# deflect-ca/banjax

Measured on AMD Instinct MI355X. Metric: log lines/sec matched+rate-limited (node) at 1k rules; HBM GB/s vs peak, higher is better.
Workload: dtype u8

## Files before the change

banjax_amd/csrc/engine.hip:

```cpp
#include <hip/hip_runtime.h>
#include <hipcub/hipcub.hpp>

#include <algorithm>
#include <array>
#include <atomic>
#include <cstdio>
#include <cstdlib>
#include <cstring>
#include <map>
#include <tuple>
#include <memory>
#include <mutex>
#include <stdexcept>
#include <string>
#include <unordered_map>
#include <thread>
#include <vector>

#include "../../include/banjax_gpu.h"
#include "bjx_common.h"
#include "engine_types.h"
#include "regex_compiler.h"
#include "bans.h"
#include "snapshot.h"
// ... 2545 lines not shown
      for (uint32_t w = w0; w < w1; ++w) {
        const uint64_t y = A[w] & cm[w];
        Yb[w] = y;
        for (uint64_t g = y & gall[w]; g; g &= g - 1) {
          const uint32_t gid = aux[w * 64u + (uint32_t)__builtin_ctzll(g)];
          atomicOr(&gmark[gid >> 5], 1u << (gid & 31));
        }
      }
      wide_sync<GLB>();
      if (s_flag) { m = true; break; }
      for (uint32_t w = w0; w < w1; ++w)
        A[w] = ((Yb[w] & sh[w]) << 1) | (w ? (Yb[w - 1] & sh[w - 1]) >> 63 : 0ull) | s0[w];
      wide_sync<GLB>();
      for (uint32_t gi = tid; gi < gw; gi += kBlock) {
        uint32_t mm = gmark[gi];
        if (!mm) continue;
        gmark[gi] = 0;
        for (; mm; mm &= mm - 1) {
          const uint32_t g = gi * 32 + (uint32_t)__ffs(mm) - 1;
          for (uint32_t q = goff[g]; q < goff[g + 1]; ++q)
            atomicOr(reinterpret_cast<unsigned long long *>(&A[gtgt[q] >> 6]), 1ull << (gtgt[q] & 63));
        }
      }
      wide_sync<GLB>();
      if (owner && (A[mw] & mbit)) s_flag = 1;
      wide_sync<GLB>();
      if (s_flag) { m = true; break; }
    }
    if (!m) {
      if (Ly.flags & kNfaAsserts) cross(ctx * 4 + 3);
      wide_sync<GLB>();
      if (owner && (A[mw] & mbit)) s_flag = 1;
      wide_sync<GLB>();
      m = s_flag != 0;
    }
    if (m && tid == 0) {
      const int32_t hid = L.host_id[j];
      atomicOr(reinterpret_cast<unsigned long long *>(&L.mword(j, pos >> 6)), 1ull << (pos & 63));
      atomicAdd(reinterpret_cast<unsigned long long *>(L.counts + j), (1ull << 32) | (is_skip(B, r, hid) ? 0ull : 1ull));
    }
    wide_sync<GLB>();
  }
}

__global__ void k_rule_bounds(uint64_t n, const uint32_t *__restrict__ jkey, uint32_t *__restrict__ first,
                              uint32_t *__restrict__ last) {
  const uint64_t i = (uint64_t)blockIdx.x * blockDim.x + threadIdx.x;
  if (i >= n) return;
  const uint32_t r = jkey[i] & 0xFFFFFF;
  if (i == 0 || (jkey[i - 1] & 0xFFFFFF) != r) first[r] = (uint32_t)i;
  if (i + 1 == n || (jkey[i + 1] & 0xFFFFFF) != r) last[r] = (uint32_t)(i + 1);
}

__global__ __launch_bounds__(kBlock) void k_emit(Bind B, uint64_t n_lines, Lines L, const uint64_t *__restrict__ offs,
                                                 uint64_t *__restrict__ res_seq, uint32_t *__restrict__ res_rule,
                                                 uint32_t *__restrict__ ev_el, uint32_t *__restrict__ ev_rule,
                                                 uint32_t *__restrict__ ev_res, unsigned long long *bounds, bool want_res) {
  __shared__ unsigned long long s_acc[2][kBlock / 64];
  unsigned long long has_ev = 0, ipb = 0;
  for (uint64_t j = (uint64_t)blockIdx.x * blockDim.x + threadIdx.x; j < n_lines; j += (uint64_t)gridDim.x * blockDim.x) {
    const uint64_t cnt = L.counts[j];
    if (cnt == 0) continue;
    uint64_t ro = offs[j] >> 32, eo = offs[j] & 0xFFFFFFFFull;
    const int32_t hid = L.host_id[j];
    uint32_t s_begin = 0, s_end = 0;
    if (hid >= 0) { s_begin = B.site_off[hid]; s_end = B.site_off[hid + 1]; }
    const uint32_t nsite = s_end - s_begin;
    const uint32_t napp = nsite + B.n_global;
    const uint32_t sc = hid >= 0 ? (uint32_t)hid : B.n_hosts;
    const uint64_t k0 = B.sc_skip[2 * sc], k1 = B.sc_skip[2 * sc + 1];
    for (uint32_t w = 0; w * 64 < napp; ++w) {
      uint64_t m = L.mword(j, w);
      while (m) {
        const uint32_t b = (uint32_t)__ffsll((unsigned long long)m) - 1;
        m &= m - 1;
        const uint32_t pos = w * 64 + b;
        const uint32_t r = pos < nsite ? B.site_rules[s_begin + pos] : B.global_rules[pos - nsite];
        const bool skip = pos < 128 ? (((pos < 64 ? k0 >> pos : k1 >> (pos - 64)) & 1) != 0) : is_skip(B, r, hid);
        if (want_res) {
          res_seq[ro] = (j << 16) | pos;
          res_rule[ro] = r | (skip ? 0x80000000u : 0u);
        }
        if (!skip) {
          ev_el[eo] = (uint32_t)j;
          ev_rule[eo] = r;
          if (want_res) ev_res[eo] = (uint32_t)ro;
          ++eo;
        }
        ++ro;
      }
    }
    if (cnt & 0xFFFFFFFFull) { ++has_ev; ipb += L.ip_len[j]; }
  }
  for (int o = 32; o > 0; o >>= 1) {
    has_ev += __shfl_xor(has_ev, o);
    ipb += __shfl_xor(ipb, o);
  }
  if ((threadIdx.x & 63) == 0) { s_acc[0][threadIdx.x >> 6] = has_ev; s_acc[1][threadIdx.x >> 6] = ipb; }
  __syncthreads();
  if (threadIdx.x == 0) {
    unsigned long long a0 = 0, a1 = 0;
    for (int w = 0; w < kBlock / 64; ++w) { a0 += s_acc[0][w]; a1 += s_acc[1][w]; }
    if (a0) { atomicAdd(&bounds[0], a0); atomicAdd(&bounds[1], a1); }
  }
}


__device__ __forceinline__ uint64_t line_start(const uint64_t *nl, uint64_t line) { return line ? nl[line - 1] + 1 : 0; }

__device__ __forceinline__ const uint8_t *ev_ip(const EvSrc &E, uint64_t i) {
  return E.bytes + (E.nl ? line_start(E.nl, i) + E.rest_off[i] - E.ip_len[i] - 1 : E.ip_pos[i]);
}
__device__ __forceinline__ uint64_t ev_hash(const EvSrc &E, uint64_t i, const uint4 &k16, uint32_t len) {
  const uint64_t h = E.nl && len <= 15 ? key16_hash(k16, len) : E.ip_hash[i];
  return E.hmask ? (h & E.hmask) | 1ull : h;
}
// ... 2203 lines not shown
  hipStream_t stream = nullptr;
  hipEvent_t ev0 = nullptr, ev1 = nullptr, evm0 = nullptr, evm1 = nullptr;
  hipEvent_t evk[4] = {};
  double kernel_ms[3] = {};
  uint32_t last_line_kernel = 0;
  static constexpr int kPhases = 8;
  hipEvent_t ph[kPhases + 1] = {};
  double phase_ms[kPhases] = {};
  hipEvent_t xev[2] = {};
  hipStream_t bstream = nullptr;
  hipEvent_t bev[kBanChunks + 1] = {};
  bool xev_rec = false;
  double exchange_ms = 0;
  bool phase_rec[kPhases + 1] = {};

  struct Entry { bool global; std::string site; int32_t decision; std::string ip; };
  std::vector<Entry> decisions;
  uint64_t decisions_version = 1;

  std::unordered_map<std::string, uint32_t> name_ids;
  std::vector<std::string> names;

  uint64_t bound_uid = 0, bound_dec_version = 0;
  DevBuf<uint8_t> bind_blob;
  Bind bind{};
  std::vector<uint4> nfa_rules;
  DevBuf<uint32_t> rb_first, rb_last;
  std::vector<uint32_t> h_first, h_last;
  std::vector<DevRule> host_rules;

  State S{};
  uint64_t ip_cap = 0, st_cap = 0;
  uint64_t ip_cap0 = 0, st_cap0 = 0, arena_cap0 = 0;
  uint64_t rehashes = 0;
  uint64_t last_new_ips = 0, last_new_states = 0;
  uint32_t epoch = 0;
  uint64_t dbg_hash_mask = 0;
  uint64_t dbg_budget = 0;
  uint32_t lines2_lds = 0;
  uint32_t lines2_w = 0;
  int dbg_slot_cache = -1;
  uint64_t host_counters[3] = {0, 0, 0};
  bool counters_fresh = false, want_counters = false;
  static constexpr uint32_t kPinBytes = 16384, kPinReads = 32;
  uint8_t *pin = nullptr;
  uint32_t pin_used = 0, pin_n = 0;
  struct PinRead { void *dst; const uint8_t *slot; uint32_t n; } pin_q[kPinReads];

  DevBuf<uint8_t> staging;
  DevBuf<uint32_t> tile_counts;
  DevBuf<uint64_t> tile_base, nl;
  DevBuf<int64_t> l_ts;
  DevBuf<uint64_t> l_iph, l_counts, l_offs, l_masks;
  DevBuf<uint32_t> l_iplen, l_roff, slow_list;
  DevBuf<int32_t> l_hid;
  DevBuf<uint64_t> l_cand;
  DevBuf<uint4> l_ip16;
  DevBuf<uint32_t> jline, jkey, jidx, jidx2, jkey2;
  DevBuf<uint64_t> jrec;
  uint64_t last_jobs = 0, last_long_runs = 0;
  DevBuf<uint64_t> long_heads;
  DevBuf<uint64_t> lr_end, lr_len, lr_off, lr_win;
  DevBuf<unsigned long long> chk;
  DevBuf<uint64_t> wide_scratch;
  DevBuf<uint32_t> wl_line, wl_rule, wl_pos;
  uint32_t wide_max_w = 0, wide_max_g = 0, n_wide = 0;
  DevBuf<uint32_t> chk_w;
  DevBuf<uint32_t> chk_wb;
  DevBuf<int64_t> lr_t0, lr_h0;
  DevBuf<uint32_t> lr_flags, lr_nwin;
  DevBuf<unsigned long long> long_count;
  DevBuf<uint32_t> bk_start, bk_big, bk_key, bk_pos;
  DevBuf<unsigned long long> bk_nbig;
  DevBuf<uint4> bk_seg;
  DevBuf<EvRec> bk_rec;
  DevBuf<uint8_t> bk_out;
  uint64_t last_big_events = 0;
  uint32_t sort2_hold = 0;
  uint64_t last_grouping = 0;
  uint32_t scan_lds[2] = {0, 0};
  bool lines_attr = false;
  DevBuf<CandMeta> l_ccnt;
  DevBuf<uint64_t> l_cfirst;
  unsigned long long scan_stats[6] = {0, 0, 0, 0, 0, 0};
  uint64_t last_slow = 0;
  DevBuf<uint8_t> l_flags;
  DevBuf<unsigned long long> scalars;
  DevBuf<uint64_t> res_seq;
  bool res_written = false;
  DevBuf<uint32_t> res_rule, ev_el, ev_rule, ev_res, ev_st, ev_st2, ev_idx, ev_idx2, el_slot, coll, trip_idx;
  DevBuf<EvRec> ev_rec, ev_rec2;
  bool rec12 = false;
  int64_t rec_base = 0;
  DevBuf<uint32_t> el_id;
  DevBuf<uint32_t> blk_n;
  DevBuf<uint64_t> blk_b;
  DevBuf<uint8_t> rl_out, ev_out, ev_out_s, trip_flag;
  DevBuf<uint32_t> trip_ev, trip_ev2;
  DevBuf<uint64_t> tr_base;
  DevBuf<bjx_trip> d_trips;
  DevBuf<bjx_rule_result> d_results;
  DevBuf<uint8_t> cub_tmp;
  DevBuf<int64_t> q_out;
  DevBuf<uint8_t> q_ip;

  BatchCtx bc;
// ... 1416 lines not shown
  S.ip_mask = cap - 1;
  (void)hipFree(S.ip_st);
  HIP_OK(hipMalloc(&S.ip_st, cap * 4));
  HIP_OK(hipMemsetAsync(S.ip_st, 0xFF, cap * 4, e->stream));
  S.ip_st_cap = cap;
  e->ip_cap = cap;
  ++e->rehashes;
}

void grow_st(bjx_engine *e, uint64_t want) {
  State &S = e->S;
  const uint64_t cap = next_pow2(want * 4 / 3 + 1024);
  if (cap <= e->st_cap) return;
  StSlot *nt;
  HIP_OK(hipMalloc(&nt, cap * sizeof(StSlot)));
  HIP_OK(hipMemsetAsync(nt, 0, cap * sizeof(StSlot), e->stream));
  hipLaunchKernelGGL(k_rehash_st, dim3(grid_for(e->st_cap)), dim3(kBlock), 0, e->stream, e->st_cap, S.st, nt, cap - 1);
  HIP_OK(hipGetLastError());
  HIP_OK(hipStreamSynchronize(e->stream));
  (void)hipFree(S.st);
  S.st = nt;
  S.st_mask = cap - 1;
  HIP_OK(hipMemsetAsync(S.ip_st, 0xFF, S.ip_st_cap * 4, e->stream));
  if (cap > (1ull << 32)) S.hot_name = kNone;
  e->st_cap = cap;
  ++e->rehashes;
}

void ensure_capacity(bjx_engine *e, uint64_t new_ips, uint64_t new_bytes, uint64_t new_states) {
  State &S = e->S;
  const uint64_t n_ips = e->host_counters[0], used = e->host_counters[1], n_st = e->host_counters[2];
  if ((n_ips + new_ips) * 4 > e->ip_cap * 3) grow_ip(e, 2 * (n_ips + new_ips));
  if (used + new_bytes > S.arena_cap) {
    const uint64_t cap = std::max<uint64_t>(S.arena_cap * 2, used + new_bytes + (1 << 20));
    uint8_t *na;
    HIP_OK(hipMalloc(&na, cap));
    HIP_OK(hipMemcpyAsync(na, S.arena, used, hipMemcpyDeviceToDevice, e->stream));
    HIP_OK(hipStreamSynchronize(e->stream));
    (void)hipFree(S.arena);
    S.arena = na;
    S.arena_cap = cap;
  }
  if ((n_st + new_states) * 4 > e->st_cap * 3) grow_st(e, 2 * (n_st + new_states));
}

template <typename F>
void cub_call(bjx_engine *e, F f) {
  size_t bytes = 0;
  HIP_OK(f((void *)nullptr, bytes));
  e->cub_tmp.ensure(bytes + 16);
  HIP_OK(f((void *)e->cub_tmp.p, bytes));
}

int bit_width(uint64_t x) {
  int b = 0;
  while (x) { ++b; x >>= 1; }
  return b;
}

}

extern "C" int bjx_engine_create(int device, const bjx_engine_options *opts, bjx_engine **out, char *err, size_t err_len) {
  if (!out) return BJX_ERR_ARG;
  *out = nullptr;
  auto e = std::make_unique<bjx_engine>();
  try {
    int n = 0;
    HIP_OK(hipGetDeviceCount(&n));
    if (device < 0 || device >= n) throw BjxError(BJX_ERR_DEVICE, "no such HIP device");
    e->device = device;
    HIP_OK(hipSetDevice(device));
    HIP_OK(hipStreamCreateWithFlags(&e->stream, hipStreamNonBlocking));
    HIP_OK(hipHostMalloc(reinterpret_cast<void **>(&e->pin), bjx_engine::kPinBytes, hipHostMallocDefault));
    HIP_OK(hipEventCreate(&e->ev0));
    HIP_OK(hipEventCreate(&e->ev1));
    HIP_OK(hipEventCreate(&e->evm0));
    HIP_OK(hipEventCreate(&e->evm1));
    for (auto &x : e->evk) HIP_OK(hipEventCreate(&x));
    for (auto &x : e->ph) HIP_OK(hipEventCreate(&x));
    for (auto &x : e->xev) HIP_OK(hipEventCreate(&x));
    uint64_t ipc = std::max<uint64_t>(opts && opts->ip_capacity ? next_pow2(opts->ip_capacity) : 0, 1ull << 22);
    uint64_t stc = std::max<uint64_t>(opts && opts->state_capacity ? next_pow2(opts->state_capacity) : 0, 1ull << 22);
    uint64_t ar = opts && opts->ip_arena_bytes ? opts->ip_arena_bytes : (64ull << 20);
    alloc_state(e.get(), ipc, stc, ar);
    e->ip_cap0 = ipc; e->st_cap0 = stc; e->arena_cap0 = ar;
    *out = e.release();
    return BJX_OK;
  } catch (const BjxError &x) {
    set_err(err, err_len, x.what());
    return x.code;
  }
}

extern "C" void bjx_engine_destroy(bjx_engine *e) {
  if (!e) return;
  (void)hipSetDevice(e->device);
  (void)hipStreamSynchronize(e->stream);
  free_state(e);
  e->trips.release(); e->trips_c.release(); e->d_trips_c.release(); e->results.release(); e->line_flags.release();
  e->ev_out_s.release(); e->trip_ev.release(); e->trip_ev2.release();
  for (auto *b : {&e->staging, &e->l_flags, &e->ev_out, &e->rl_out, &e->trip_flag, &e->bind_blob,
                  &e->cub_tmp, &e->q_ip})
    b->release();
  e->tile_counts.release(); e->tile_base.release(); e->nl.release(); e->l_ts.release(); e->l_iph.release();
  e->l_counts.release(); e->l_offs.release(); e->l_masks.release(); e->l_iplen.release();
  e->l_roff.release(); e->slow_list.release(); e->l_hid.release();
  e->scalars.release(); e->res_seq.release(); e->res_rule.release(); e->ev_el.release(); e->ev_rule.release();

  e->ev_res.release(); e->ev_st.release(); e->ev_st2.release(); e->ev_idx.release(); e->ev_idx2.release();
  e->el_slot.release(); e->coll.release(); e->blk_n.release(); e->blk_b.release(); e->ev_rec.release(); e->ev_rec2.release(); e->el_id.release();

  for (auto *b : {&e->pack_src, &e->rx_len, &e->rx_ev_el}) b->release();
  for (auto *b : {&e->pk_hist, &e->pk_off, &e->pk_counts, &e->pk_bbase, &e->rx_hash, &e->rx_pos, &e->rx_nev, &e->rx_evoff})
    b->release();
  e->rx_ts.release(); e->rx_ip16.release(); e->trip_idx.release(); e->d_trips.release(); e->tr_base.release();
  for (auto *b : {&e->bn_key, &e->bn_key2, &e->bn_len, &e->bn_off, &e->dl_hash}) b->release();
  for (auto *b : {&e->bn_val, &e->bn_val2, &e->bn_head, &e->bn_seg, &e->bn_first, &e->bn_cnt, &e->bn_ipt, &e->bn_coll,
                  &e->dl_off, &e->dl_len, &e->nm_off})
    b->release();
  for (auto *b : {&e->bn_kind, &e->bn_flag, &e->bn_log, &e->dl_bytes, &e->nm_json}) b->release();
  e->bn_best.release(); e->bn_rep.release(); e->bn_sel.release(); e->bn_ipb.release(); e->tz_at.release(); e->tz_off.release();
  e->rb_first.release(); e->rb_last.release(); e->long_heads.release(); e->long_count.release();
  e->lr_end.release(); e->lr_len.release(); e->lr_off.release(); e->lr_win.release(); e->lr_t0.release(); e->lr_h0.release();
  e->lr_flags.release(); e->lr_nwin.release(); e->chk.release(); e->chk_w.release(); e->chk_wb.release();
  for (auto *b : {&e->bk_start, &e->bk_big, &e->bk_key, &e->bk_pos}) b->release();
  e->bk_nbig.release(); e->bk_seg.release(); e->bk_rec.release(); e->bk_out.release();
  e->d_results.release(); e->q_out.release();
  e->ban_ips.release(); e->ban_log.release(); e->ban_off.release(); e->ban_kind.release(); e->ban_ipb.release();
  e->ban_ipo.release();
  e->snap_pin.release();
  e->qry_rows.release();
  e->qry_bytes.release();
  e->l_ip16.release(); e->jline.release(); e->jkey.release(); e->jidx.release(); e->jidx2.release(); e->jrec.release(); e->jkey2.release(); e->l_cand.release(); e->l_ccnt.release(); e->l_cfirst.release();
  (void)hipEventDestroy(e->ev0); (void)hipEventDestroy(e->ev1); (void)hipEventDestroy(e->evm0); (void)hipEventDestroy(e->evm1);
  for (auto &x : e->evk) (void)hipEventDestroy(x);
  for (auto &x : e->ph) (void)hipEventDestroy(x);
  for (auto &x : e->xev) (void)hipEventDestroy(x);
  for (auto &x : e->bev) if (x) (void)hipEventDestroy(x);
  if (e->bstream) (void)hipStreamDestroy(e->bstream);
  (void)hipStreamDestroy(e->stream);
  if (e->pin) (void)hipHostFree(e->pin);
  delete e;
}

extern "C" const char *bjx_engine_last_error(bjx_engine *e) { return e ? e->last_error.c_str() : "no engine"; }

extern "C" int bjx_engine_set_decision_lists(bjx_engine *e, const bjx_decision_entry *entries, size_t n) {
  if (!e || (n && !entries)) return BJX_ERR_ARG;
  std::lock_guard<std::mutex> g(e->mu);
  std::vector<bjx_engine::Entry> v;
  for (size_t i = 0; i < n; ++i) {
    if (entries[i].decision < BJX_ALLOW || entries[i].decision > BJX_IPTABLES_BLOCK) return BJX_ERR_DECISION;
    bjx_engine::Entry x;
    x.global = entries[i].site.ptr == nullptr;
    if (!x.global) x.site.assign(entries[i].site.ptr, entries[i].site.len);
    x.decision = entries[i].decision;
    x.ip.assign(entries[i].ip.ptr ? entries[i].ip.ptr : "", entries[i].ip.len);
    v.push_back(std::move(x));
// ... 376 lines not shown
    const uint8_t *sp = bytes;
    if (flags & BJX_INPUT_DEVICE) {
      sample.resize(sn);
      if (sn) HIP_OK(hipMemcpy(sample.data(), bytes, sn, hipMemcpyDeviceToHost));
      sp = sample.data();
    }
    bind_ruleset(e, rs, sp, sn);
  }
  const Bind &B = e->bind;
  hipStream_t st = e->stream;
  memset(out, 0, sizeof *out);
  e->trips.clear();
  e->trips_c.clear();
  e->results.clear();
  e->line_flags.clear();
  if (n == 0) return false;

  const uint8_t *buf = bytes;
  if (!(flags & BJX_INPUT_DEVICE) || (reinterpret_cast<uintptr_t>(bytes) & 15)) {
    e->staging.ensure(n + 16);
    HIP_OK(hipMemcpyAsync(e->staging.p, bytes, n, (flags & BJX_INPUT_DEVICE) ? hipMemcpyDeviceToDevice : hipMemcpyHostToDevice, st));
    buf = e->staging.p;
  }
  HIP_OK(hipEventRecord(e->ev0, st));
  for (auto &r : e->phase_rec) r = false;
  mark(e, 0);

  const uint64_t n_tiles = (n + kWT - 1) / kWT;
  e->tile_counts.ensure(n_tiles);
  e->tile_base.ensure(n_tiles + 1);
  uint64_t n_lines = 0;
  Lines L;
  hipLaunchKernelGGL(k_nl_count_wt, dim3((unsigned)((n_tiles + 3) / 4)), dim3(kBlock), 0, st, buf, (uint64_t)n, n_tiles,
                     e->tile_counts.p);
  HIP_OK(hipGetLastError());
  {
    uint32_t *in = e->tile_counts.p;
    uint64_t *o = e->tile_base.p;
    cub_call(e, [&](void *tmp, size_t &bytes) { return hipcub::DeviceScan::ExclusiveSum(tmp, bytes, in, o, (int)n_tiles, st); });
  }
  {
    uint64_t last_base = 0;
    uint32_t last_cnt = 0;
    pin_get(e, &last_base, e->tile_base.p + (n_tiles - 1), 8);
    pin_get(e, &last_cnt, e->tile_counts.p + (n_tiles - 1), 4);
    pin_sync(e);
    n_lines = last_base + last_cnt;
  }
  out->n_lines = n_lines;
  if (n_lines == 0) return false;
  const uint64_t cap = n_lines;

  e->nl.ensure(cap);
  e->l_ts.ensure(cap); e->l_iph.ensure(cap); e->l_counts.ensure(cap + 1); e->l_offs.ensure(cap + 1);
  e->l_masks.ensure(cap * B.mask_words);
  e->l_iplen.ensure(cap);
  e->l_roff.ensure(cap); e->l_hid.ensure(cap); e->l_flags.ensure(cap); e->slow_list.ensure(cap);
  e->l_ccnt.ensure(cap); e->l_ip16.ensure(cap);
  e->l_cand.ensure(B.any_prefilter ? cap * kCandSlots : 1);
  e->scalars.ensure(16);
  L.ts = e->l_ts.p; L.ip_hash = e->l_iph.p; L.ip_len = e->l_iplen.p;
  L.rest_off = e->l_roff.p; L.host_id = e->l_hid.p; L.flags = e->l_flags.p;
  L.counts = e->l_counts.p; L.masks = e->l_masks.p; L.mstride = cap;
  L.cand_meta = e->l_ccnt.p; L.cand = e->l_cand.p; L.ip16 = e->l_ip16.p;
  L.cand_first = nullptr;
  if (B.cfirst) {
    e->l_cfirst.ensure(cap * kCandFirstLits);
    L.cand_first = e->l_cfirst.p;
    HIP_OK(hipMemsetAsync(e->l_cfirst.p, 0xFF, cap * kCandFirstLits * 8, st));
  }
  e->jline.ensure(std::max<uint64_t>(e->jline.n, cap + (1u << 20)));
  e->jkey.ensure(e->jline.n); e->jidx.ensure(e->jline.n); e->jrec.ensure(e->jline.n);
  HIP_OK(hipMemsetAsync(e->scalars.p, 0, 16 * sizeof(unsigned long long), st));
  if (B.any_prefilter) HIP_OK(hipMemsetAsync(e->l_ccnt.p, 0, cap * sizeof(CandMeta), st));
  mark(e, 1);

  {
    int n_cu_scan = 0;
    HIP_OK(hipDeviceGetAttribute(&n_cu_scan, hipDeviceAttributeMultiprocessorCount, e->device));
    const unsigned scan_grid = (unsigned)std::min<uint64_t>((n_tiles + kScanWaves - 1) / kScanWaves, (uint64_t)std::max(1, n_cu_scan));
    ScanArgs A;
    A.buf = buf; A.n = n; A.n_tiles = n_tiles; A.n_lines = cap; A.tile_base = e->tile_base.p; A.nl = e->nl.p;
    A.L = L; A.stats = e->scalars.p + 8;
    A.debug_skip = getenv("BJX_DEBUG_SKIP") ? (uint32_t)atoi(getenv("BJX_DEBUG_SKIP")) : 0u;
    const uint32_t fixed = kPairBytes + kScanWaves * kWaveLds;
    const bool img_lds = fixed + B.scan_img_bytes <= kScanLdsMax;
    A.shared_bytes = img_lds ? B.scan_img_bytes : 0;
    const uint32_t lds = A.shared_bytes + kScanWaves * kWaveLds;
    using ScanFn = void (*)(Bind, ScanArgs);
    const ScanFn kfn = img_lds ? k_scan<true> : k_scan<false>;
    if (lds != e->scan_lds[img_lds]) {
      HIP_OK(hipFuncSetAttribute(reinterpret_cast<const void *>(kfn), hipFuncAttributeMaxDynamicSharedMemorySize, (int)lds));
      e->scan_lds[img_lds] = lds;
    }
    HIP_OK(hipEventRecord(e->evm0, st));
    hipLaunchKernelGGL(kfn, dim3(scan_grid), dim3(kScanWaves * 64), lds, st, B, A);
    HIP_OK(hipGetLastError());
    HIP_OK(hipEventRecord(e->evm1, st));
  }
  uint64_t last_nl = 0;
  mark(e, 2);

  unsigned long long sc4[5] = {0, 0, 0, 0, 0};
  unsigned long long n_jobs = 0;
  const bool all_wide = B.n_global > 128 && !(getenv("BJX_LINES") && atoi(getenv("BJX_LINES")) == 1);
  int n_cu = 0;
  HIP_OK(hipDeviceGetAttribute(&n_cu, hipDeviceAttributeMultiprocessorCount, e->device));
// ... 172 lines not shown
        const uint32_t r = k % B.n_rules;
        if (l[k] <= f[k]) continue;
        by_rx[r < rs->rules.size() ? rs->rules[r].regex.substr(0, 60) : "?"] += l[k] - f[k];
        if (k >= B.n_rules) n_legacy += l[k] - f[k];
      }
      std::vector<std::pair<uint64_t, std::string>> v;
      for (auto &kv : by_rx) v.push_back({kv.second, kv.first});
      std::sort(v.rbegin(), v.rend());
      fprintf(stderr, "BJX_JOB_STATS jobs=%llu (legacy %llu) lines=%llu\n", n_jobs, (unsigned long long)n_legacy,
              (unsigned long long)e->bc.n_lines);
      for (size_t i = 0; i < v.size() && i < 16; ++i) fprintf(stderr, "  %10llu  %s\n", (unsigned long long)v[i].first, v[i].second.c_str());
    }
  }
  HIP_OK(hipEventRecord(e->evk[3], st));
  if (n_slow) {
    WideList WL{nullptr, nullptr, nullptr, e->scalars.p + 13, 0};
    if (B.any_wide) {
      const uint64_t cap = n_slow * (uint64_t)e->n_wide + 1;
      e->wl_line.ensure(cap); e->wl_rule.ensure(cap); e->wl_pos.ensure(cap);
      WL.line = e->wl_line.p; WL.rule = e->wl_rule.p; WL.pos = e->wl_pos.p; WL.cap = cap;
      HIP_OK(hipMemsetAsync(e->scalars.p + 13, 0, 8, st));
    }
    if (all_wide) HIP_OK(hipEventRecord(e->evk[0], st));
    hipLaunchKernelGGL(k_parse_match<true>, dim3(grid_for(n_slow)), dim3(kBlock), 0, st, B, buf, e->nl.p, (uint64_t)n_slow,
                       all_wide ? nullptr : e->slow_list.p, now_ns, L, e->slow_list.p, e->scalars.p, WL);
    HIP_OK(hipGetLastError());
    if (B.any_wide) {
      unsigned long long n_wl = 0;
      pin_get(e, &n_wl, e->scalars.p + 13, 8);
      pin_sync(e);
      if (n_wl > WL.cap) throw BjxError(BJX_ERR_DEVICE, "internal: wide-NFA job list overflow");
      if (n_wl) launch_wide(e, B, buf, n, e->wl_rule.p, nullptr, e->wl_line.p, e->wl_pos.p, 0, n_wl, L, e->wide_max_w, e->wide_max_g);
    }
    if (all_wide) HIP_OK(hipEventRecord(e->evk[1], st));
  }
  e->last_slow = n_slow;
  if (getenv("BJX_CHECK")) {
    e->chk.ensure(16);
    HIP_OK(hipMemsetAsync(e->chk.p, 0, 16, st));
    hipLaunchKernelGGL(k_check_masks, dim3(grid_for(n_lines)), dim3(kBlock), 0, st, n_lines, L, B.mask_words, e->chk.p);
    HIP_OK(hipGetLastError());
    unsigned long long c[2];
    pin_get(e, c, e->chk.p, 16);
    pin_sync(e);
    if (c[0]) {
      char msg[160];
      snprintf(msg, sizeof msg, "BJX_CHECK: %llu lines whose RuleResult count differs from their match mask (first %llu)", c[0],
               c[1]);
      throw BjxError(BJX_ERR_DEVICE, msg);
    }
  }
  mark(e, 3);

  HIP_OK(hipMemsetAsync(e->l_counts.p + n_lines, 0, 8, st));
  {
    uint64_t *in = e->l_counts.p, *o = e->l_offs.p;
    cub_call(e, [&](void *tmp, size_t &bytes) {
      return hipcub::DeviceScan::ExclusiveSum(tmp, bytes, in, o, (int)(n_lines + 1), st);
    });
  }
  uint64_t tot = 0;
  pin_get(e, &tot, e->l_offs.p + n_lines, 8);
  pin_sync(e);
  const uint64_t n_res = tot >> 32, n_ev = tot & 0xFFFFFFFFull;
  out->n_results = n_res;
  out->n_events = n_ev;
  e->res_seq.ensure(n_res + 1); e->res_rule.ensure(n_res + 1); e->rl_out.ensure(n_res + 1);
  e->ev_el.ensure(n_ev + 1); e->ev_rule.ensure(n_ev + 1); e->ev_res.ensure(n_ev + 1);
  HIP_OK(hipMemsetAsync(e->scalars.p + 1, 0, 2 * 8, st));
  e->res_written = false;
  if (n_res) {
    const bool want_res = (flags & BJX_COPY_RESULTS) != 0;
    e->res_written = want_res;
    hipLaunchKernelGGL(k_emit, dim3((unsigned)std::min<uint64_t>(grid_for(n_lines), 4096)), dim3(kBlock), 0, st, B, n_lines, L,
                       e->l_offs.p, e->res_seq.p, e->res_rule.p, e->ev_el.p, e->ev_rule.p, e->ev_res.p, e->scalars.p + 1,
                       e->res_written);
    HIP_OK(hipGetLastError());
    if (e->res_written) HIP_OK(hipMemsetAsync(e->rl_out.p, 0, n_res, st));
  }
  mark(e, 4);
  unsigned long long bnd[2] = {0, 0};
  if (n_ev) {
    pin_get(e, bnd, e->scalars.p + 1, 16);
    if (e->want_counters) pin_get(e, e->host_counters, e->S.counters, 24);
    pin_sync(e);
    e->counters_fresh = e->want_counters;
  }
  BatchCtx &c = e->bc;
  c.buf = buf; c.n_lines = n_lines; c.n_res = n_res; c.n_ev = n_ev; c.L = L; c.n_el = bnd[0]; c.el_bytes = bnd[1];
  c.consumed = out->consumed_bytes;
  c.now_ns = now_ns;
  c.live = true;
  return true;
}

static EvSrc local_evsrc(bjx_engine *e) {
  const BatchCtx &c = e->bc;
  EvSrc E;
  E.bytes = c.buf; E.nl = e->nl.p; E.rest_off = c.L.rest_off; E.ip_pos = nullptr; E.ip_len = c.L.ip_len;
  E.ip_hash = c.L.ip_hash; E.ts = c.L.ts; E.counts = c.L.counts; E.ip16 = c.L.ip16; E.n = c.n_lines;
  E.hmask = e->dbg_hash_mask;
  return E;
}

static void ensure_name_json(bjx_engine *e) {
  if (e->nm_built == e->names.size() && e->nm_off.p) return;
  std::vector<uint32_t> off;
  std::vector<uint8_t> js;
  for (const auto &nm : e->names) {
    off.push_back((uint32_t)js.size());
    const uint8_t *b = reinterpret_cast<const uint8_t *>(nm.data());
    JOut<false> c{nullptr, 0};
    json_str(c, b, (uint32_t)nm.size());
    const size_t at = js.size();
    js.resize(at + c.n);
    JOut<true> w{js.data() + at, 0};
    json_str(w, b, (uint32_t)nm.size());
  }
  off.push_back((uint32_t)js.size());
  e->nm_off.ensure(off.size());
  e->nm_json.ensure(js.size() + 16);
  HIP_OK(hipMemcpy(e->nm_off.p, off.data(), off.size() * 4, hipMemcpyHostToDevice));
  if (!js.empty()) HIP_OK(hipMemcpy(e->nm_json.p, js.data(), js.size(), hipMemcpyHostToDevice));
  e->nm_built = e->names.size();
}

__global__ void k_ban_iplen(BanDev A, uint64_t n_ips, const bjx_ip_decision *__restrict__ sel, uint64_t *__restrict__ len) {
  const uint64_t i = (uint64_t)blockIdx.x * blockDim.x + threadIdx.x;
// ... 150 lines not shown
  if (from == kFinSorted)
    hipLaunchKernelGGL(k_trip_events, dim3(grid_for(n_trips)), dim3(kBlock), 0, st, n_trips, e->trip_idx.p, ev_words(e),
                       rec_stride(e), e->trip_ev.p);
  uint32_t *ki = from == kFinSorted ? e->trip_ev.p : e->trip_idx.p, *ko = e->trip_ev2.p;
  const int bits = std::max(1, bit_width(n_ev));
  cub_call(e, [&](void *tmp, size_t &bytes) {
    return hipcub::DeviceRadixSort::SortKeys(tmp, bytes, ki, ko, (int)n_trips, 0, bits, st);
  });
  if (from == kFinList && n_trips > 1) {
    HIP_OK(hipMemsetAsync(e->scalars.p + 6, 0, 8, st));
    hipLaunchKernelGGL(k_count_dups, dim3(grid_for(n_trips)), dim3(kBlock), 0, st, n_trips, ko, e->scalars.p + 6);
    HIP_OK(hipGetLastError());
    unsigned long long dups = 0;
    pin_get(e, &dups, e->scalars.p + 6, 8);
    pin_sync(e);
    if (dups) throw BjxError(BJX_ERR_ARG, "bjx_finish_batch_trips: an event index appears more than once");
  }
  return n_trips;
}

static void finish_phase(bjx_engine *e, uint32_t flags, bjx_batch_result *out, FinishFrom from, uint64_t n_list = 0) {
  const Bind &B = e->bind;
  hipStream_t st = e->stream;
  const BatchCtx &c = e->bc;
  const uint64_t n_lines = c.n_lines, n_res = c.n_res, n_ev = c.n_ev;
  const Lines &L = c.L;
  uint64_t n_trips = 0;
  e->ban_emitted = (flags & BJX_EMIT_BANS) != 0;
  e->ban_n_trips = 0;
  e->ban_ips.resize(0); e->ban_log.resize(0); e->ban_off.resize(1); e->ban_off.data()[0] = 0; e->ban_kind.resize(0);
  e->ban_ipb.resize(0); e->ban_ipo.resize(1); e->ban_ipo.data()[0] = 0;
  if (n_ev) {
    mark(e, 7);
    n_trips = trip_events(e, n_ev, from, n_list);
    if (n_trips) {
      e->d_trips.ensure(n_trips);
      hipLaunchKernelGGL(k_build_trips, dim3(grid_for(n_trips)), dim3(kBlock), 0, st, n_trips, e->trip_ev2.p, e->ev_el.p,
                         e->ev_rule.p, c.buf, e->nl.p, L, B.rules, e->d_trips.p);
      HIP_OK(hipGetLastError());
      if (flags & BJX_TRIPS_COMPACT) {
        e->d_trips_c.ensure(n_trips);
        hipLaunchKernelGGL(k_pack_trips, dim3(grid_for(n_trips)), dim3(kBlock), 0, st, n_trips, e->d_trips.p, e->d_trips_c.p);
        HIP_OK(hipGetLastError());
        e->trips_c.resize(n_trips);
        HIP_OK(hipMemcpyAsync(e->trips_c.data(), e->d_trips_c.p, n_trips * 8, hipMemcpyDeviceToHost, st));
      } else {
        e->trips.resize(n_trips);
        HIP_OK(hipMemcpyAsync(e->trips.data(), e->d_trips.p, n_trips * sizeof(bjx_trip), hipMemcpyDeviceToHost, st));
      }
      if (flags & BJX_EMIT_BANS) emit_bans(e, n_trips, (flags & BJX_BAN_RECORDS_ONLY) != 0);
    }
    if ((flags & BJX_COPY_RESULTS) && !e->res_written) {
      HIP_OK(hipMemsetAsync(e->scalars.p + 1, 0, 2 * 8, st));
      hipLaunchKernelGGL(k_emit, dim3((unsigned)std::min<uint64_t>(grid_for(n_lines), 4096)), dim3(kBlock), 0, st, e->bind,
                         n_lines, L, e->l_offs.p, e->res_seq.p, e->res_rule.p, e->ev_el.p, e->ev_rule.p, e->ev_res.p,
                         e->scalars.p + 1, true);
      HIP_OK(hipGetLastError());
      HIP_OK(hipMemsetAsync(e->rl_out.p, 0, n_res, st));
      e->res_written = true;
    }
    if (flags & BJX_COPY_RESULTS) {
      if (from == kFinSorted)
        hipLaunchKernelGGL(k_unsort, dim3(grid_for(n_ev)), dim3(kBlock), 0, st, n_ev, ev_words(e), rec_stride(e), e->ev_out_s.p,
                           e->ev_out.p);
      hipLaunchKernelGGL(k_scatter_rl, dim3(grid_for(n_ev)), dim3(kBlock), 0, st, n_ev, e->ev_res.p, e->ev_out.p, e->rl_out.p);
      HIP_OK(hipGetLastError());
      if (getenv("BJX_CHECK")) {
        e->chk_w.ensure(n_res + 1);
        e->chk.ensure(16);
        HIP_OK(hipMemsetAsync(e->chk_w.p, 0, (n_res + 1) * 4, st));
        HIP_OK(hipMemsetAsync(e->chk.p, 0, 32, st));
        hipLaunchKernelGGL(k_check_count, dim3(grid_for(n_ev)), dim3(kBlock), 0, st, n_ev, e->ev_res.p, 1u, n_res, e->chk_w.p,
                           e->chk.p);
        hipLaunchKernelGGL(k_check_most, dim3(grid_for(n_res)), dim3(kBlock), 0, st, n_res, e->chk_w.p, 1u, e->chk.p);
        HIP_OK(hipGetLastError());
        unsigned long long c[3];
        pin_get(e, c, e->chk.p, 24);
        pin_sync(e);
        if (c[0] || c[1]) {
          char msg[256];
          snprintf(msg, sizeof msg, "BJX_CHECK: %llu event result indices out of range, %llu RuleResults named by more than "
                   "one event (first %llu)", c[0], c[1], c[2]);
          throw BjxError(BJX_ERR_DEVICE, msg);
        }
      }
    }
  }
  HIP_OK(hipEventRecord(e->ev1, st));
  mark(e, 8);
  if (flags & BJX_COPY_RESULTS) {
    hipLaunchKernelGGL(k_final_flags, dim3(grid_for(n_lines)), dim3(kBlock), 0, st, n_lines, e->l_flags.p);
    e->line_flags.resize(n_lines);
    HIP_OK(hipMemcpyAsync(e->line_flags.data(), e->l_flags.p, n_lines, hipMemcpyDeviceToHost, st));
    if (n_res) {
      e->d_results.ensure(n_res);
      hipLaunchKernelGGL(k_build_results, dim3(grid_for(n_res)), dim3(kBlock), 0, st, n_res, e->res_seq.p, e->res_rule.p,
                         e->rl_out.p, e->d_results.p);
      e->results.resize(n_res);
      HIP_OK(hipMemcpyAsync(e->results.data(), e->d_results.p, n_res * sizeof(bjx_rule_result), hipMemcpyDeviceToHost, st));
    }
  }
  HIP_OK(hipStreamSynchronize(st));
  float ms = 0, mms = 0;
  HIP_OK(hipEventElapsedTime(&ms, e->ev0, e->ev1));
  HIP_OK(hipEventElapsedTime(&mms, e->evm0, e->evm1));
  {
    float kl = 0, kd = 0;
    HIP_OK(hipEventElapsedTime(&kl, e->evk[0], e->evk[1]));
// ... 1350 lines not shown
```

Before: 2.616 billion.

## Derive emit offsets from per-tile sums and in-block scans, not a per-line scan

A new kernel computes one count sum per tile of lines, and a small device scan over those tile sums gives each tile's base offset. The emit kernel then rebuilds each line's result/event offset with a wavefront shuffle scan plus a shared-memory per-wave prefix, and reads the batch total from the tile scan. The goal is to drop the full-length per-line exclusive scan and its l_offs array traffic. However, the full per-line scan is still run when counters are not requested, which is probably the default path, so that path gains an extra kernel and scan. The grid cap can now also be set through an environment variable.

Result: no change. 2.635 billion (median of 6 runs) (+0.7%).

```diff
diff --git a/banjax_amd/csrc/engine.hip b/banjax_amd/csrc/engine.hip
--- a/banjax_amd/csrc/engine.hip
+++ b/banjax_amd/csrc/engine.hip
@@ -2621,16 +2621,46 @@
   if (i + 1 == n || (jkey[i + 1] & 0xFFFFFF) != r) last[r] = (uint32_t)(i + 1);
 }
 
-__global__ __launch_bounds__(kBlock) void k_emit(Bind B, uint64_t n_lines, Lines L, const uint64_t *__restrict__ offs,
+__global__ __launch_bounds__(kBlock) void k_count_tiles(uint64_t n_lines, const uint64_t *__restrict__ counts,
+                                                        uint64_t *__restrict__ tile_sums) {
+  __shared__ unsigned long long s_w[kBlock / 64];
+  const uint64_t j = (uint64_t)blockIdx.x * kBlock + threadIdx.x;
+  uint64_t v = j < n_lines ? counts[j] : 0;
+#pragma unroll
+  for (int d = 32; d >= 1; d >>= 1) v += __shfl_xor(v, d);
+  if ((threadIdx.x & 63) == 0) s_w[threadIdx.x >> 6] = v;
+  __syncthreads();
+  if (threadIdx.x == 0) {
+    for (int w = 1; w < kBlock / 64; ++w) v += s_w[w];
+    tile_sums[blockIdx.x] = v;
+  }
+}
+
+__global__ __launch_bounds__(kBlock) void k_emit(Bind B, uint64_t n_lines, Lines L, const uint64_t *__restrict__ tile_base,
                                                  uint64_t *__restrict__ res_seq, uint32_t *__restrict__ res_rule,
                                                  uint32_t *__restrict__ ev_el, uint32_t *__restrict__ ev_rule,
                                                  uint32_t *__restrict__ ev_res, unsigned long long *bounds, bool want_res) {
   __shared__ unsigned long long s_acc[2][kBlock / 64];
+  __shared__ unsigned long long s_pre[2][kBlock / 64];
   unsigned long long has_ev = 0, ipb = 0;
-  for (uint64_t j = (uint64_t)blockIdx.x * blockDim.x + threadIdx.x; j < n_lines; j += (uint64_t)gridDim.x * blockDim.x) {
-    const uint64_t cnt = L.counts[j];
+  const uint32_t lane = threadIdx.x & 63, wave = threadIdx.x >> 6;
+  const uint64_t n_tiles = (n_lines + kBlock - 1) / kBlock;
+  uint32_t trip = 0;
+  for (uint64_t t = blockIdx.x; t < n_tiles; t += gridDim.x, trip ^= 1) {
+    const uint64_t j = t * kBlock + threadIdx.x;
+    const uint64_t cnt = j < n_lines ? L.counts[j] : 0;
+    uint64_t x = cnt;
+#pragma unroll
+    for (int d = 1; d < 64; d <<= 1) {
+      const uint64_t y = __shfl_up(x, d);
+      if (lane >= (uint32_t)d) x += y;
+    }
+    if (lane == 63) s_pre[trip][wave] = x;
+    __syncthreads();
     if (cnt == 0) continue;
-    uint64_t ro = offs[j] >> 32, eo = offs[j] & 0xFFFFFFFFull;
+    uint64_t off = tile_base[t] + x - cnt;
+    for (uint32_t w = 0; w < wave; ++w) off += s_pre[trip][w];
+    uint64_t ro = off >> 32, eo = off & 0xFFFFFFFFull;
     const int32_t hid = L.host_id[j];
     uint32_t s_begin = 0, s_end = 0;
     if (hid >= 0) { s_begin = B.site_off[hid]; s_end = B.site_off[hid + 1]; }
@@ -4940,6 +4970,7 @@
   DevBuf<uint64_t> tile_base, nl;
   DevBuf<int64_t> l_ts;
   DevBuf<uint64_t> l_iph, l_counts, l_offs, l_masks;
+  DevBuf<uint64_t> emit_sums, emit_base;
   DevBuf<uint32_t> l_iplen, l_roff, slow_list;
   DevBuf<int32_t> l_hid;
   DevBuf<uint64_t> l_cand;
@@ -6462,6 +6493,12 @@
   HIP_OK(f((void *)e->cub_tmp.p, bytes));
 }
 
+unsigned emit_grid(uint64_t n_lines) {
+  const char *cap_env = getenv("BJX_EMIT_GRID");
+  const uint64_t cap = cap_env && atoll(cap_env) > 0 ? (uint64_t)atoll(cap_env) : 4096ull;
+  return (unsigned)std::min<uint64_t>((n_lines + kBlock - 1) / kBlock, cap);
+}
+
 int bit_width(uint64_t x) {
   int b = 0;
   while (x) { ++b; x >>= 1; }
@@ -6514,6 +6551,7 @@
     b->release();
   e->tile_counts.release(); e->tile_base.release(); e->nl.release(); e->l_ts.release(); e->l_iph.release();
   e->l_counts.release(); e->l_offs.release(); e->l_masks.release(); e->l_iplen.release();
+  e->emit_sums.release(); e->emit_base.release();
   e->l_roff.release(); e->slow_list.release(); e->l_hid.release();
   e->scalars.release(); e->res_seq.release(); e->res_rule.release(); e->ev_el.release(); e->ev_rule.release();
 
@@ -6996,7 +7034,7 @@
   const uint64_t cap = n_lines;
 
   e->nl.ensure(cap);
-  e->l_ts.ensure(cap); e->l_iph.ensure(cap); e->l_counts.ensure(cap + 1); e->l_offs.ensure(cap + 1);
+  e->l_ts.ensure(cap); e->l_iph.ensure(cap); e->l_counts.ensure(cap + 1);
   e->l_masks.ensure(cap * B.mask_words);
   e->l_iplen.ensure(cap);
   e->l_roff.ensure(cap); e->l_hid.ensure(cap); e->l_flags.ensure(cap); e->slow_list.ensure(cap);
@@ -7275,15 +7313,27 @@
   }
   mark(e, 3);
 
-  HIP_OK(hipMemsetAsync(e->l_counts.p + n_lines, 0, 8, st));
+  const uint64_t n_et = (n_lines + kBlock - 1) / kBlock;
+  e->emit_sums.ensure(n_et + 1); e->emit_base.ensure(n_et + 1);
+  hipLaunchKernelGGL(k_count_tiles, dim3((unsigned)n_et), dim3(kBlock), 0, st, n_lines, e->l_counts.p, e->emit_sums.p);
+  HIP_OK(hipGetLastError());
+  HIP_OK(hipMemsetAsync(e->emit_sums.p + n_et, 0, 8, st));
   {
+    uint64_t *in = e->emit_sums.p, *o = e->emit_base.p;
+    cub_call(e, [&](void *tmp, size_t &bytes) {
+      return hipcub::DeviceScan::ExclusiveSum(tmp, bytes, in, o, (int)(n_et + 1), st);
+    });
+  }
+  if (!e->want_counters) {
+    e->l_offs.ensure(n_lines + 1);
+    HIP_OK(hipMemsetAsync(e->l_counts.p + n_lines, 0, 8, st));
     uint64_t *in = e->l_counts.p, *o = e->l_offs.p;
     cub_call(e, [&](void *tmp, size_t &bytes) {
       return hipcub::DeviceScan::ExclusiveSum(tmp, bytes, in, o, (int)(n_lines + 1), st);
     });
   }
   uint64_t tot = 0;
-  pin_get(e, &tot, e->l_offs.p + n_lines, 8);
+  pin_get(e, &tot, e->emit_base.p + n_et, 8);
   pin_sync(e);
   const uint64_t n_res = tot >> 32, n_ev = tot & 0xFFFFFFFFull;
   out->n_results = n_res;
@@ -7295,8 +7345,7 @@
   if (n_res) {
     const bool want_res = (flags & BJX_COPY_RESULTS) != 0;
     e->res_written = want_res;
-    hipLaunchKernelGGL(k_emit, dim3((unsigned)std::min<uint64_t>(grid_for(n_lines), 4096)), dim3(kBlock), 0, st, B, n_lines, L,
-                       e->l_offs.p, e->res_seq.p, e->res_rule.p, e->ev_el.p, e->ev_rule.p, e->ev_res.p, e->scalars.p + 1,
+    hipLaunchKernelGGL(k_emit, dim3(emit_grid(n_lines)), dim3(kBlock), 0, st, B, n_lines, L, e->emit_base.p, e->res_seq.p, e->res_rule.p, e->ev_el.p, e->ev_rule.p, e->ev_res.p, e->scalars.p + 1,
                        e->res_written);
     HIP_OK(hipGetLastError());
     if (e->res_written) HIP_OK(hipMemsetAsync(e->rl_out.p, 0, n_res, st));
@@ -7553,8 +7602,7 @@
     }
     if ((flags & BJX_COPY_RESULTS) && !e->res_written) {
       HIP_OK(hipMemsetAsync(e->scalars.p + 1, 0, 2 * 8, st));
-      hipLaunchKernelGGL(k_emit, dim3((unsigned)std::min<uint64_t>(grid_for(n_lines), 4096)), dim3(kBlock), 0, st, e->bind,
-                         n_lines, L, e->l_offs.p, e->res_seq.p, e->res_rule.p, e->ev_el.p, e->ev_rule.p, e->ev_res.p,
+      hipLaunchKernelGGL(k_emit, dim3(emit_grid(n_lines)), dim3(kBlock), 0, st, e->bind, n_lines, L, e->emit_base.p, e->res_seq.p, e->res_rule.p, e->ev_el.p, e->ev_rule.p, e->ev_res.p,
                          e->scalars.p + 1, true);
       HIP_OK(hipGetLastError());
       HIP_OK(hipMemsetAsync(e->rl_out.p, 0, n_res, st));
```
